# libAudioFlux/audioFlux

Hardware: NVIDIA H100
Metric: mfcc_frames_per_s (higher is better)
Workload: dtype f32

## Files before the change

### audioflux_b200/csrc/gen/gen_fft32.py

```python
#!/usr/bin/env python3
import math
import sys

import numpy as np


def bitrev5(k):
    return int("{:05b}".format(k)[::-1], 2)


def build_ops(n=32):
    ops = []
    span = n // 2
    while span >= 1:
        for base in range(0, n, 2 * span):
            for j in range(span):
                theta = 2 * math.pi * j / (2 * span)
                c, s = math.cos(theta), math.sin(theta)
                if j == 0:
                    kind = "one"
                elif 2 * j == span:
                    kind = "mi"
                elif 4 * j == span:
                    kind = "w8_1"
# ... 16 lines not shown
    bits = n.bit_length() - 1
    for i, j, kind, c, s in build_ops(n):
        u, v = x[i], x[j]
        x[i] = u + v
        x[j] = (u - v) * complex(c, -s)
    out = np.empty(n, dtype=np.complex128)
    for k in range(n):
        out[k] = x[bitrev(k, bits)]
    return out


def selfcheck():
    rng = np.random.default_rng(0)
    err = 0.0
    for n in (16, 32):
        x = rng.standard_normal(n) + 1j * rng.standard_normal(n)
        err = max(err, np.abs(run_numpy(x) - np.fft.fft(x)).max())
    x = rng.standard_normal(32) + 1j * rng.standard_normal(32)
    err = max(err, np.abs(run_numpy_fma(x) - np.fft.fft(x)).max())
    s = rng.standard_normal(64)
    err = max(err, np.abs(run_numpy_rfft64(s / 2) - np.fft.rfft(s)).max())
    w = rng.standard_normal(32) + 1j * rng.standard_normal(32)
    err = max(err, np.abs(run_numpy_fma_win(x, w) - np.fft.fft(x.real * w.real + 1j * x.imag * w.imag)).max())
    g, t = np.ones(32), np.zeros(32)
    for j in range(1, 32):
        g[j], t[j] = twiddle_gt(17 * j)
    err = max(err, np.abs(run_numpy_fma_tw(x, g, t) - np.fft.fft(x * g * (1 - 1j * t))).max())
    assert err < 1e-12, err
    return err


def lit(v):
    return repr(float(np.float32(v))) + "f"


def emit():
    out = []
    w = out.append
    w("// GENERATED by gen/gen_fft32.py -- do not edit.  32-point forward DFT on registers,")
    w("// complex values packed as c64 (see c64.cuh); X[k] is left at index AF_BR5(k) (5-bit reversal).")
    w("#pragma once")
    w('#include "c64.cuh"')
    w("#define AF_BR5(k) ((((k) & 1) << 4) | (((k) & 2) << 2) | ((k) & 4) | (((k) & 8) >> 2) | (((k) & 16) >> 4))")
    w("#define AF_BR4(k) ((((k) & 1) << 3) | (((k) & 2) << 1) | (((k) & 4) >> 1) | (((k) & 8) >> 3))")
    r2 = lit(math.sqrt(0.5))
    for n in (32, 16):
# ... 131 lines not shown
    for k in range(n // 4):
        mi1, g1, t1 = _twiddle(2 * math.pi * k / n)
        mi3, g3, t3 = _twiddle(2 * math.pi * 3 * k / n)
        a = o.rot(z1[k], t1)
        b = o.rot(z3[k], t3)
        if mi1:
            a = _mul_mi(a)
        if mi3:
            b = _mul_mi(b)
        if abs(g1) >= abs(g3):
            G, r = g1, _snap(g3 / g1)
            s, d = o.clin(b, r, a), o.clin(b, -r, a)
        else:
            G, r = g3, _snap(g1 / g3)
            s, d = o.clin(a, r, b), o.clin(a, r, (_neg(b[0]), _neg(b[1])))
        md = _mul_mi(d)
        out[k] = o.clin(s, G, u[k])
        out[k + n // 2] = o.clin(s, -G, u[k])
        out[k + n // 4] = o.clin(md, G, u[k + n // 4])
        out[k + 3 * n // 4] = o.clin(md, -G, u[k + n // 4])
    return out


def _inputs(n):
    return [((f"x{j}r", 1), (f"x{j}i", 1)) for j in range(n)]


def build_fma_fft32():
    o = _Ops()
    return o.ops, _split_radix(o, _inputs(32))


def build_fma_post64():
    o = _Ops()
    z = _inputs(32)
    out = [None] * 32
    for k in range(1, 16):
        zk, zc = z[k], (z[32 - k][0], _neg(z[32 - k][1]))
        ev = o.clin(zc, 1.0, zk)
        od = o.clin(zc, -1.0, zk)
        mi, g, t = _twiddle(2 * math.pi * k / 64 + math.pi / 2)
        a = o.rot(od, t)
        if mi:
            a = _mul_mi(a)
        out[k] = o.clin(a, g, ev)
        out[32 - k] = (o.lin(a[0], -g, ev[0]), o.lin(a[1], g, _neg(ev[1])))
    out[16] = (o.mul(z[16][0], 2.0), o.mul(z[16][1], -2.0))
    out[0] = (o.mul(o.lin(z[0][1], 1.0, z[0][0]), 2.0), o.mul(o.lin(z[0][1], -1.0, z[0][0]), 2.0))
    return o.ops, out


def build_fma_fft32_win():
    o = _Ops()
    xs = [((f"x{j}r", 1, f"w{j}r"), (f"x{j}i", 1, f"w{j}i")) for j in range(32)]
    return o.ops, _split_radix(o, xs)


def build_fma_fft32_tw():
    o = _Ops()
    xs = [((f"x0r", 1), (f"x0i", 1))]
    for j in range(1, 32):
        re = o.fmar((f"x{j}i", 1), f"t{j}", (f"x{j}r", 1))
        im = o.fmar((f"x{j}r", -1), f"t{j}", (f"x{j}i", 1))
        xs.append((re + (f"g{j}",), im + (f"g{j}",)))
    return o.ops, _split_radix(o, xs)


def twiddle_gt(m, n=2048):
    th = 2 * math.pi * m / n
    return math.cos(th), math.tan(th)


def fp32_op_count(ops):
    return len(ops)


def run_ops(ops, outs, x, dtype=np.float64, regs=None):
    f = np.float64 if dtype == np.float64 else np.float32
    env = {k: f(v) for k, v in (regs or {}).items()}
    for j, v in enumerate(x):
# ... 30 lines not shown
def run_numpy_fma_win(x, w, dtype=np.float64):
    ops, outs = build_fma_fft32_win()
    w = np.asarray(w, dtype=np.complex128)
    regs = {}
    for j in range(32):
        regs[f"w{j}r"], regs[f"w{j}i"] = w[j].real, w[j].imag
    return run_ops(ops, outs, np.asarray(x, dtype=np.complex128), dtype, regs)


def run_numpy_fma_tw(x, g, t, dtype=np.float64):
    ops, outs = build_fma_fft32_tw()
    regs = {}
    for j in range(1, 32):
        regs[f"g{j}"], regs[f"t{j}"] = g[j], t[j]
    return run_ops(ops, outs, np.asarray(x, dtype=np.complex128), dtype, regs)


def run_numpy_rfft64(s, dtype=np.float64):
    s = np.asarray(s, dtype=np.float64)
    x = s[0::2] + 1j * s[1::2]
    Z = run_numpy_fma(x, dtype)
    ops, outs = build_fma_post64()
    R = run_ops(ops, outs, Z, dtype)
    return np.concatenate([[R[0].real], R[1:32], [R[0].imag]])


def _operand(a):
    return ("-" if a[1] < 0 else "") + a[0]


def _emit_ops(w, ops):
    for op in ops:
        if op[0] == "add":
            a, b = op[2], op[3]
            if a[1] > 0 and b[1] < 0:
                w(f"    const float {op[1]} = __fsub_rn({a[0]}, {b[0]});")
            elif a[1] < 0 and b[1] > 0:
                w(f"    const float {op[1]} = __fsub_rn({b[0]}, {a[0]});")
            else:
                w(f"    const float {op[1]} = __fadd_rn({_operand(a)}, {_operand(b)});")
        elif op[0] == "mul":
            k = op[3] * op[2][1]
            w(f"    const float {op[1]} = __fmul_rn({op[2][0]}, {lit(k)});")
        elif op[0] == "mulr":
            w(f"    const float {op[1]} = __fmul_rn({_operand(op[2])}, {op[3]});")
        elif op[0] == "fmar":
# ... 3 lines not shown
            w(f"    const float {op[1]} = __fmaf_rn({op[2][0]}, {lit(k)}, {_operand(op[4])});")


def emit_fma():
    out = []
    w = out.append
    w("")
    w("// ---- FMA-oriented transforms (scalar FP32, one instruction per op; only the fused MFCC frame path uses them) ----")
    w("// Twiddles as u g (1 - i t), |t| <= 1, g folded into the consumer's FMAs; +-i and negation are operand modifiers.")
    w("// Results differ from af_fft32 in the last bits (different rounding sequence), deterministic.")
    ops, outs = build_fma_fft32()
    w("// Split-radix (decimation in time) 32-point forward DFT; X[k] is left at index AF_BR5(k), as af_fft32 leaves it.")
    w("__device__ __forceinline__ void af_fft32_fma(c64 (&z)[32]) {")
    for j in range(32):
        w(f"    float x{j}r, x{j}i; c_unpack(z[{j}], x{j}r, x{j}i);")
    _emit_ops(w, ops)
    for k, (r, i) in enumerate(outs):
        assert r[1] > 0 and i[1] > 0
        w(f"    z[{bitrev5(k)}] = c_pack({r[0]}, {i[0]});")
    w("}")
    w(f"// af_fft32_fma FP32 instruction count: {fp32_op_count(ops)}")
    ops, outs = build_fma_fft32_win()
    w("// af_fft32_fma of the windowed input (z[j].re w[32 j].re, z[j].im w[32 j].im): the window factors are applied inside")
    w("// the first butterflies (one FMUL + two FMAs per butterfly and component).")
    w("__device__ __forceinline__ void af_fft32_fma_win(c64 (&z)[32], const c64 *w) {")
    for j in range(32):
        w(f"    float x{j}r, x{j}i, w{j}r, w{j}i; c_unpack(z[{j}], x{j}r, x{j}i); c_unpack(w[{32 * j}], w{j}r, w{j}i);")
    _emit_ops(w, ops)
    for k, (r, i) in enumerate(outs):
        assert r[1] > 0 and i[1] > 0
        w(f"    z[{bitrev5(k)}] = c_pack({r[0]}, {i[0]});")
    w("}")
    w(f"// af_fft32_fma_win FP32 instruction count: {fp32_op_count(ops)}")
    ops, outs = build_fma_fft32_tw()
    w("// af_fft32_fma of z[j] g_j (1 - i t_j), (g_j, t_j) = tw[32 (j - 1)] for j = 1..31 (input 0 is taken as it is):")
    w("// two FMAs apply (1 - i t), g goes into the first butterflies as af_fft32_fma_win's window factors do.")
    w("__device__ __forceinline__ void af_fft32_fma_tw(c64 (&z)[32], const c64 *tw) {")
    w("    float x0r, x0i; c_unpack(z[0], x0r, x0i);")
    for j in range(1, 32):
        w(f"    float x{j}r, x{j}i, g{j}, t{j}; c_unpack(z[{j}], x{j}r, x{j}i); c_unpack(tw[{32 * (j - 1)}], g{j}, t{j});")
    _emit_ops(w, ops)
    for k, (r, i) in enumerate(outs):
        assert r[1] > 0 and i[1] > 0
        w(f"    z[{bitrev5(k)}] = c_pack({r[0]}, {i[0]});")
    w("}")
    w(f"// af_fft32_fma_tw FP32 instruction count: {fp32_op_count(ops)}")
    ops, outs = build_fma_post64()
    w("// Real 64-point DFT post-pass on the output of af_fft32_fma (Z[k] at AF_BR5(k)): R[k] at AF_BR5(k) for k = 1..31,")
    w("// (R[0], R[32]) packed at index 0; the window carries the factor 1/2.")
    w("__device__ __forceinline__ void af_rfft64_post_fma(c64 (&z)[32]) {")
    for j in range(32):
        w(f"    float x{j}r, x{j}i; c_unpack(z[{bitrev5(j)}], x{j}r, x{j}i);")
    _emit_ops(w, ops)
    for k, (r, i) in enumerate(outs):
        assert r[1] > 0 and i[1] > 0
        w(f"    z[{bitrev5(k)}] = c_pack({r[0]}, {i[0]});")
    w("}")
    w(f"// af_rfft64_post_fma FP32 instruction count: {fp32_op_count(ops)}")
    return out


if __name__ == "__main__":
    e = selfcheck()
    path = sys.argv[1] if len(sys.argv) > 1 else "../kernels/fft32_gen.cuh"
    with open(path, "w") as f:
        f.write(emit())
    n_r2 = sum(2 if kind in ("one", "mi") else 4 for _, _, kind, _, _ in build_ops(32))
    print(f"selfcheck err {e:.2e}; wrote {path}; FP32 instructions: af_fft32 {2 * n_r2}, "
          f"af_fft32_fma {fp32_op_count(build_fma_fft32()[0])}, af_fft32_fma_win {fp32_op_count(build_fma_fft32_win()[0])}, "
          f"af_fft32_fma_tw {fp32_op_count(build_fma_fft32_tw()[0])}, af_rfft64_post_fma {fp32_op_count(build_fma_post64()[0])}")
```

### audioflux_b200/csrc/kernels/fft32_gen.cuh

```cuda
#pragma once
#include "c64.cuh"
#define AF_BR5(k) ((((k) & 1) << 4) | (((k) & 2) << 2) | ((k) & 4) | (((k) & 8) >> 2) | (((k) & 16) >> 4))
#define AF_BR4(k) ((((k) & 1) << 3) | (((k) & 2) << 1) | (((k) & 4) >> 1) | (((k) & 8) >> 3))
__device__ __forceinline__ void af_fft32(c64 (&z)[32]) {
    c64 u, d;
    u = z[0]; d = c_sub(u, z[16]); z[0] = c_add(u, z[16]);
    z[16] = d;
    u = z[1]; d = c_sub(u, z[17]); z[1] = c_add(u, z[17]);
    z[17] = c_mul_cs(d, 0.9807852506637573f, 0.19509032368659973f);
    u = z[2]; d = c_sub(u, z[18]); z[2] = c_add(u, z[18]);
    z[18] = c_mul_cs(d, 0.9238795042037964f, 0.3826834261417389f);
    u = z[3]; d = c_sub(u, z[19]); z[3] = c_add(u, z[19]);
    z[19] = c_mul_cs(d, 0.8314695954322815f, 0.5555702447891235f);
    u = z[4]; d = c_sub(u, z[20]); z[4] = c_add(u, z[20]);
    z[20] = c_scale(c_add(d, c_mul_mi(d)), 0.7071067690849304f);
    u = z[5]; d = c_sub(u, z[21]); z[5] = c_add(u, z[21]);
    z[21] = c_mul_cs(d, 0.5555702447891235f, 0.8314695954322815f);
    u = z[6]; d = c_sub(u, z[22]); z[6] = c_add(u, z[22]);
    z[22] = c_mul_cs(d, 0.3826834261417389f, 0.9238795042037964f);
    u = z[7]; d = c_sub(u, z[23]); z[7] = c_add(u, z[23]);
    z[23] = c_mul_cs(d, 0.19509032368659973f, 0.9807852506637573f);
    u = z[8]; d = c_sub(u, z[24]); z[8] = c_add(u, z[24]);
    z[24] = c_mul_mi(d);
    u = z[9]; d = c_sub(u, z[25]); z[9] = c_add(u, z[25]);
// ... 1887 lines not shown
    z[10] = c_pack(v97, v98);
    z[26] = c_pack(v107, v108);
    z[6] = c_pack(v117, v118);
    z[22] = c_pack(v127, v128);
    z[14] = c_pack(v137, v138);
    z[30] = c_pack(v147, v148);
    z[1] = c_pack(v151, v152);
    z[17] = c_pack(v149, v150);
    z[9] = c_pack(v139, v140);
    z[25] = c_pack(v129, v130);
    z[5] = c_pack(v119, v120);
    z[21] = c_pack(v109, v110);
    z[13] = c_pack(v99, v100);
    z[29] = c_pack(v89, v90);
    z[3] = c_pack(v79, v80);
    z[19] = c_pack(v69, v70);
    z[11] = c_pack(v59, v60);
    z[27] = c_pack(v49, v50);
    z[7] = c_pack(v39, v40);
    z[23] = c_pack(v29, v30);
    z[15] = c_pack(v19, v20);
    z[31] = c_pack(v9, v10);
}
```

### audioflux_b200/csrc/kernels/mfcc_fused2.cu

```cuda
#include <string.h>
#include "mfcc_common.cuh"
#include "fft32_gen.cuh"

namespace {

constexpr int kN = 2048;
constexpr int kBins = 1025;
constexpr int kPairs = 513;
constexpr int kFW = 13;
constexpr int kBW = 4;
constexpr int kDW = 2;
constexpr int kEW = kBW;
constexpr int kThreads = (kFW + 1 + kBW + kDW) * 32;
constexpr int kProducerWarp = 13;
__device__ __forceinline__ int bank_warp_index(int warp) { return warp >= 14 && warp <= 18 && warp != 16 ? warp - 14 - (warp > 16) : -1; }
__device__ __forceinline__ int dct_warp_index(int warp) { return warp == 16 || warp == 19 ? (warp - 16) / 3 : -1; }
constexpr int kMaxNum = 128;
constexpr int kLPitch = 132;
constexpr int kMaxTab = 1408;
constexpr int kMaxPieces = 256;
constexpr int kMaxPass = kMaxPieces / (kEW * 32);
constexpr int kSpecPitch = 17;
constexpr int kPitchPairs = kFW | 1;
constexpr int kTileFloats = kPairs * kPitchPairs * 2;
// ... 366 lines not shown
        float *col = sP + sb * kTileFloats + 2 * warp;

        af_mbar_wait(&fullBar[stage], stagePhase);

        c64 z[32];
        if (active) {
            const float *sp = span + (size_t)stage * p.spanFloats + warp * p.hop + lane;
#pragma unroll
            for (int m = 0; m < 32; m++) z[m] = c_pack(sp[64 * m], sp[64 * m + 32]);
        }
        __syncwarp();
        if (lane == 0) af_mbar_arrive(&emptyBar[stage]);
        if (++stage == p.stages) { stage = 0; stagePhase ^= 1u; }
        if (!active) {
            af_mbar_wait(&pEmpty[sb], ((uint32_t)(it >> 1) & 1u) ^ 1u);
            if (lane == 0) {
                af_mbar_arrive(&specFull[sb]);
                af_mbar_arrive(&cDone[sb]);
                af_mbar_arrive(&pFull[sb]);
            }
            continue;
        }

        af_fft32_fma_win(z, sWinC + lane);
        af_rfft64_post_fma(z);
        af_mbar_wait(&pEmpty[sb], ((uint32_t)(it >> 1) & 1u) ^ 1u);
        sSpec[((size_t)sb * 32 + lane) * kSpecPitch + warp] = z[0];
        __syncwarp();
        if (lane == 0) af_mbar_arrive(&specFull[sb]);

        {
            float yr[32], yi[32];
            float *tw = col + trWrite;
            const float2 *row = reinterpret_cast<const float2 *>(col) + trRead;
#pragma unroll
            for (int k1 = 1; k1 < 32; k1++) c_unpack(z[AF_BR5(k1)], yr[k1], yi[k1]);
#pragma unroll
            for (int k1 = 1; k1 < 32; k1++) tw[(k1 - 1) * 2 * pitch] = yr[k1];
            __syncwarp();
#pragma unroll
            for (int j = 0; j < 16; j++) { const float2 v = row[j * kTrRows * pitch]; yr[2 * j] = v.x; yr[2 * j + 1] = v.y; }
            __syncwarp();
#pragma unroll
            for (int k1 = 1; k1 < 32; k1++) tw[(k1 - 1) * 2 * pitch] = yi[k1];
            __syncwarp();
#pragma unroll
            for (int j = 0; j < 16; j++) {
                const float2 v = row[j * kTrRows * pitch];
                z[2 * j] = c_pack(yr[2 * j], v.x);
                z[2 * j + 1] = c_pack(yr[2 * j + 1], v.y);
            }
            __syncwarp();
            if (lane == 0) af_mbar_arrive(&cDone[sb]);
        }
        af_fft32_fma_tw(z, sTwC + lane);
        if (lane) {
            if (p.dataType == SpectralData_Mag) {
#pragma unroll
                for (int k2 = 0; k2 < 32; k2++) {
// ... 179 lines not shown
    Intervals *iv = static_cast<Intervals *>(malloc(sizeof(Intervals)));
    float4 *tab = static_cast<float4 *>(malloc(sizeof(float4) * kMaxTab));
    unsigned desc[kMaxNum + 4];
    PiecePlan *pc = static_cast<PiecePlan *>(malloc(sizeof(PiecePlan)));
    const int ok = iv && tab && pc && build_intervals2(bank, num, iv) && build_table(bank, num, iv, desc, tab) >= 0 &&
                   plan_pieces(num, desc, pc) > 0;
    free(iv); free(tab); free(pc);
    return ok;
}

void af_mfcc2_plan_free(void *plan) { free_plan(static_cast<Plan *>(plan)); }

int af_mfcc2_plan_build(void **planOut, int fftLength, int num, int ccNum, const float *window, const float *bank,
                        const float *dct , int dataType) {
    *planOut = NULL;
    if (!af_mfcc2_supported(fftLength, num, ccNum, bank)) return af_fail(AF_ERR_UNSUPPORTED, "fused MFCC v2 plan: unsupported configuration");
    Plan *pl = static_cast<Plan *>(calloc(1, sizeof(Plan)));
    if (!pl) return AF_ERR_NOMEM;
    pl->num = num; pl->ccNum = ccNum; pl->dataType = dataType;
    pl->ct = af_mfcc_ct(ccNum);
    int rc = AF_OK;

    float2 *wp = static_cast<float2 *>(malloc(sizeof(float2) * 1024));
    for (int m = 0; m < 32; m++)
        for (int l = 0; l < 32; l++) wp[m * 32 + l] = make_float2(0.5f * window[64 * m + l], 0.5f * window[64 * m + 32 + l]);
    rc = af_dev_upload(reinterpret_cast<void **>(&pl->dWinPairs), wp, sizeof(float2) * 1024);
    for (int n2 = 1; n2 <= kTwRows; n2++)
        for (int k1 = 0; k1 < 32; k1++) {
            const double a = 2.0 * M_PI * (double)(n2 * k1) / 2048.0;
            wp[(n2 - 1) * 32 + k1] = make_float2((float)cos(a), (float)tan(a));
        }
    if (rc == AF_OK) rc = af_dev_upload(reinterpret_cast<void **>(&pl->dTw), wp, sizeof(float2) * kTwRows * 32);
    free(wp);

    Intervals *iv = static_cast<Intervals *>(malloc(sizeof(Intervals)));
    pl->tab = static_cast<float4 *>(malloc(sizeof(float4) * kMaxTab));
    if (!iv || !pl->tab) { free(iv); free_plan(pl); return AF_ERR_NOMEM; }
    build_intervals2(bank, num, iv);
    pl->tabLen = build_table(bank, num, iv, pl->ivDesc, pl->tab);
    free(iv);
    for (int i = num + 2; i < kMaxNum + 4; i++) pl->ivDesc[i] = pl->ivDesc[num + 1];
    {
        PiecePlan *pc = static_cast<PiecePlan *>(malloc(sizeof(PiecePlan)));
        if (!pc || plan_pieces(num, pl->ivDesc, pc) <= 0) { free(pc); free_plan(pl); return af_fail(AF_ERR_UNSUPPORTED, "fused MFCC v2 plan: no piece plan"); }
        pl->nPass = pc->nPass; pl->nPieces = pc->nPieces; pl->lmax = pc->lmax; pl->firstPass2 = pc->firstPass2;
        memcpy(pl->pieceDesc, pc->pieceDesc, sizeof(pl->pieceDesc));
        memcpy(pl->piecePrefix, pc->prefix, sizeof(pl->piecePrefix));
        memcpy(pl->assign, pc->assign, sizeof(pl->assign));
// ... 83 lines not shown
```

Before: 240.2 million.

## Replace packed complex FFT32 plus real post-pass with direct split-radix real FFT64

Stage B of the fused MFCC kernel used to run a 32-point complex FFT on packed sample pairs followed by a separate real-64 post-pass. It now runs one generated split-radix real 64-point DFT with the window applied inside the first butterflies, and writes outputs in natural order so the transpose no longer needs bit-reversed indexing. The aim is fewer FP32 instructions and lower register pressure in the per-warp FFT. The window-pair table layout on the host changes to match, and rounding differs slightly from the old path.

```diff
diff --git a/audioflux_b200/csrc/gen/gen_fft32.py b/audioflux_b200/csrc/gen/gen_fft32.py
--- a/audioflux_b200/csrc/gen/gen_fft32.py
+++ b/audioflux_b200/csrc/gen/gen_fft32.py
@@ -62,6 +62,8 @@
     err = max(err, np.abs(run_numpy_rfft64(s / 2) - np.fft.rfft(s)).max())
     w = rng.standard_normal(32) + 1j * rng.standard_normal(32)
     err = max(err, np.abs(run_numpy_fma_win(x, w) - np.fft.fft(x.real * w.real + 1j * x.imag * w.imag)).max())
+    w = rng.standard_normal(64)
+    err = max(err, np.abs(run_numpy_rfft64_win(s, w) - np.fft.rfft(s * w)).max())
     g, t = np.ones(32), np.zeros(32)
     for j in range(1, 32):
         g[j], t[j] = twiddle_gt(17 * j)
@@ -239,6 +241,48 @@
     return out
 
 
+def _real_split_radix(o, xs):
+    n = len(xs)
+    if n == 1:
+        return [xs[0]]
+    if n == 2:
+        return [o.lin(xs[1], 1.0, xs[0]), o.lin(xs[1], -1.0, xs[0])]
+    u = _real_split_radix(o, xs[0::2])
+    z1 = _real_split_radix(o, xs[1::4])
+    z3 = _real_split_radix(o, xs[3::4])
+    out = [None] * (n // 2 + 1)
+    a, nb = o.lin(z1[0], 1.0, z3[0]), o.lin(z1[0], -1.0, z3[0])
+    out[0], out[n // 2] = o.lin(a, 1.0, u[0]), o.lin(a, -1.0, u[0])
+    out[n // 4] = (u[n // 4], nb)
+    if n >= 8:
+        e, r = n // 8, math.sqrt(0.5)
+        p, q = o.lin(z3[e], -1.0, z1[e]), o.lin(z3[e], 1.0, z1[e])
+        ue = u[e]
+        out[e] = (o.lin(p, r, ue[0]), o.lin(q, -r, ue[1]))
+        out[3 * e] = (o.lin(p, -r, ue[0]), o.lin(q, -r, _neg(ue[1])))
+    for k in range(1, n // 8):
+        mi1, g1, t1 = _twiddle(2 * math.pi * k / n)
+        mi3, g3, t3 = _twiddle(2 * math.pi * 3 * k / n)
+        a = o.rot(z1[k], t1)
+        b = o.rot(z3[k], t3)
+        if mi1:
+            a = _mul_mi(a)
+        if mi3:
+            b = _mul_mi(b)
+        if abs(g1) >= abs(g3):
+            G, r = g1, _snap(g3 / g1)
+            s, d = o.clin(b, r, a), o.clin(b, -r, a)
+        else:
+            G, r = g3, _snap(g1 / g3)
+            s, d = o.clin(a, r, b), o.clin(a, r, (_neg(b[0]), _neg(b[1])))
+        uk, uq = u[k], u[n // 4 - k]
+        out[k] = o.clin(s, G, uk)
+        out[n // 2 - k] = (o.lin(s[0], -G, uk[0]), o.lin(s[1], G, _neg(uk[1])))
+        out[n // 4 + k] = (o.lin(d[1], G, uq[0]), o.lin(d[0], -G, _neg(uq[1])))
+        out[n // 4 - k] = (o.lin(d[1], -G, uq[0]), o.lin(d[0], -G, uq[1]))
+    return out
+
+
 def _inputs(n):
     return [((f"x{j}r", 1), (f"x{j}i", 1)) for j in range(n)]
 
@@ -273,6 +317,13 @@
     return o.ops, _split_radix(o, xs)
 
 
+def build_fma_rfft64_win():
+    o = _Ops()
+    xs = [(f"x{n // 2}{'ri'[n & 1]}", 1, f"w{n}") for n in range(64)]
+    R = _real_split_radix(o, xs)
+    return o.ops, [(R[0], R[32])] + R[1:32]
+
+
 def build_fma_fft32_tw():
     o = _Ops()
     xs = [((f"x0r", 1), (f"x0i", 1))]
@@ -349,6 +400,14 @@
     Z = run_numpy_fma(x, dtype)
     ops, outs = build_fma_post64()
     R = run_ops(ops, outs, Z, dtype)
+    return np.concatenate([[R[0].real], R[1:32], [R[0].imag]])
+
+
+def run_numpy_rfft64_win(s, w, dtype=np.float64):
+    ops, outs = build_fma_rfft64_win()
+    s, w = np.asarray(s, dtype=np.float64), np.asarray(w, dtype=np.float64)
+    regs = {f"w{n}": w[n] for n in range(64)}
+    R = run_ops(ops, outs, s[0::2] + 1j * s[1::2], dtype, regs)
     return np.concatenate([[R[0].real], R[1:32], [R[0].imag]])
 
 
@@ -398,7 +457,8 @@
     w(f"// af_fft32_fma FP32 instruction count: {fp32_op_count(ops)}")
     ops, outs = build_fma_fft32_win()
     w("// af_fft32_fma of the windowed input (z[j].re w[32 j].re, z[j].im w[32 j].im): the window factors are applied inside")
-    w("// the first butterflies (one FMUL + two FMAs per butterfly and component).")
+    w("// the first butterflies (one FMUL + two FMAs per butterfly and component).  With af_rfft64_post_fma it makes the real")
+    w("// 64-point DFT of packed sample pairs; no kernel calls the pair now (the fused MFCC stage B is af_rfft64_fma_win).")
     w("__device__ __forceinline__ void af_fft32_fma_win(c64 (&z)[32], const c64 *w) {")
     for j in range(32):
         w(f"    float x{j}r, x{j}i, w{j}r, w{j}i; c_unpack(z[{j}], x{j}r, x{j}i); c_unpack(w[{32 * j}], w{j}r, w{j}i);")
@@ -423,7 +483,8 @@
     w(f"// af_fft32_fma_tw FP32 instruction count: {fp32_op_count(ops)}")
     ops, outs = build_fma_post64()
     w("// Real 64-point DFT post-pass on the output of af_fft32_fma (Z[k] at AF_BR5(k)): R[k] at AF_BR5(k) for k = 1..31,")
-    w("// (R[0], R[32]) packed at index 0; the window carries the factor 1/2.")
+    w("// (R[0], R[32]) packed at index 0; the window carries the factor 1/2.  Not called by any kernel now (see")
+    w("// af_fft32_fma_win).")
     w("__device__ __forceinline__ void af_rfft64_post_fma(c64 (&z)[32]) {")
     for j in range(32):
         w(f"    float x{j}r, x{j}i; c_unpack(z[{bitrev5(j)}], x{j}r, x{j}i);")
@@ -433,6 +494,19 @@
         w(f"    z[{bitrev5(k)}] = c_pack({r[0]}, {i[0]});")
     w("}")
     w(f"// af_rfft64_post_fma FP32 instruction count: {fp32_op_count(ops)}")
+    ops, outs = build_fma_rfft64_win()
+    w("// Split-radix (decimation in time) real 64-point DFT of the windowed samples s[n] w[n], packed as z[j] = (s[2j],")
+    w("// s[2j+1]), with the window pairs w[32 n] = (w[n], w[n + 32]) of the first butterflies (s[n] with s[n + 32]); the")
+    w("// window factors are applied inside them.  Leaves R[k] at z[k] for k = 1..31 and the real pair (R[0], R[32]) at z[0].")
+    w("__device__ __forceinline__ void af_rfft64_fma_win(c64 (&z)[32], const c64 *w) {")
+    for j in range(32):
+        w(f"    float x{j}r, x{j}i, w{j}, w{j + 32}; c_unpack(z[{j}], x{j}r, x{j}i); c_unpack(w[{32 * j}], w{j}, w{j + 32});")
+    _emit_ops(w, ops)
+    for k, (r, i) in enumerate(outs):
+        assert r[1] > 0 and i[1] > 0
+        w(f"    z[{k}] = c_pack({r[0]}, {i[0]});")
+    w("}")
+    w(f"// af_rfft64_fma_win FP32 instruction count: {fp32_op_count(ops)}")
     return out
 
 
@@ -444,4 +518,5 @@
     n_r2 = sum(2 if kind in ("one", "mi") else 4 for _, _, kind, _, _ in build_ops(32))
     print(f"selfcheck err {e:.2e}; wrote {path}; FP32 instructions: af_fft32 {2 * n_r2}, "
           f"af_fft32_fma {fp32_op_count(build_fma_fft32()[0])}, af_fft32_fma_win {fp32_op_count(build_fma_fft32_win()[0])}, "
-          f"af_fft32_fma_tw {fp32_op_count(build_fma_fft32_tw()[0])}, af_rfft64_post_fma {fp32_op_count(build_fma_post64()[0])}")
+          f"af_fft32_fma_tw {fp32_op_count(build_fma_fft32_tw()[0])}, af_rfft64_post_fma {fp32_op_count(build_fma_post64()[0])}, "
+          f"af_rfft64_fma_win {fp32_op_count(build_fma_rfft64_win()[0])}")
diff --git a/audioflux_b200/csrc/kernels/fft32_gen.cuh b/audioflux_b200/csrc/kernels/fft32_gen.cuh
--- a/audioflux_b200/csrc/kernels/fft32_gen.cuh
+++ b/audioflux_b200/csrc/kernels/fft32_gen.cuh
@@ -1933,3 +1933,495 @@
     z[15] = c_pack(v19, v20);
     z[31] = c_pack(v9, v10);
 }
+__device__ __forceinline__ void af_rfft64_fma_win(c64 (&z)[32], const c64 *w) {
+    float x0r, x0i, w0, w32; c_unpack(z[0], x0r, x0i); c_unpack(w[0], w0, w32);
+    float x1r, x1i, w1, w33; c_unpack(z[1], x1r, x1i); c_unpack(w[32], w1, w33);
+    float x2r, x2i, w2, w34; c_unpack(z[2], x2r, x2i); c_unpack(w[64], w2, w34);
+    float x3r, x3i, w3, w35; c_unpack(z[3], x3r, x3i); c_unpack(w[96], w3, w35);
+    float x4r, x4i, w4, w36; c_unpack(z[4], x4r, x4i); c_unpack(w[128], w4, w36);
+    float x5r, x5i, w5, w37; c_unpack(z[5], x5r, x5i); c_unpack(w[160], w5, w37);
+    float x6r, x6i, w6, w38; c_unpack(z[6], x6r, x6i); c_unpack(w[192], w6, w38);
+    float x7r, x7i, w7, w39; c_unpack(z[7], x7r, x7i); c_unpack(w[224], w7, w39);
+    float x8r, x8i, w8, w40; c_unpack(z[8], x8r, x8i); c_unpack(w[256], w8, w40);
+    float x9r, x9i, w9, w41; c_unpack(z[9], x9r, x9i); c_unpack(w[288], w9, w41);
+    float x10r, x10i, w10, w42; c_unpack(z[10], x10r, x10i); c_unpack(w[320], w10, w42);
+    float x11r, x11i, w11, w43; c_unpack(z[11], x11r, x11i); c_unpack(w[352], w11, w43);
+    float x12r, x12i, w12, w44; c_unpack(z[12], x12r, x12i); c_unpack(w[384], w12, w44);
+    float x13r, x13i, w13, w45; c_unpack(z[13], x13r, x13i); c_unpack(w[416], w13, w45);
+    float x14r, x14i, w14, w46; c_unpack(z[14], x14r, x14i); c_unpack(w[448], w14, w46);
+    float x15r, x15i, w15, w47; c_unpack(z[15], x15r, x15i); c_unpack(w[480], w15, w47);
+    float x16r, x16i, w16, w48; c_unpack(z[16], x16r, x16i); c_unpack(w[512], w16, w48);
+    float x17r, x17i, w17, w49; c_unpack(z[17], x17r, x17i); c_unpack(w[544], w17, w49);
+    float x18r, x18i, w18, w50; c_unpack(z[18], x18r, x18i); c_unpack(w[576], w18, w50);
+    float x19r, x19i, w19, w51; c_unpack(z[19], x19r, x19i); c_unpack(w[608], w19, w51);
+    float x20r, x20i, w20, w52; c_unpack(z[20], x20r, x20i); c_unpack(w[640], w20, w52);
+    float x21r, x21i, w21, w53; c_unpack(z[21], x21r, x21i); c_unpack(w[672], w21, w53);
+    float x22r, x22i, w22, w54; c_unpack(z[22], x22r, x22i); c_unpack(w[704], w22, w54);
+    float x23r, x23i, w23, w55; c_unpack(z[23], x23r, x23i); c_unpack(w[736], w23, w55);
+    float x24r, x24i, w24, w56; c_unpack(z[24], x24r, x24i); c_unpack(w[768], w24, w56);
+    float x25r, x25i, w25, w57; c_unpack(z[25], x25r, x25i); c_unpack(w[800], w25, w57);
+    float x26r, x26i, w26, w58; c_unpack(z[26], x26r, x26i); c_unpack(w[832], w26, w58);
+    float x27r, x27i, w27, w59; c_unpack(z[27], x27r, x27i); c_unpack(w[864], w27, w59);
+    float x28r, x28i, w28, w60; c_unpack(z[28], x28r, x28i); c_unpack(w[896], w28, w60);
+    float x29r, x29i, w29, w61; c_unpack(z[29], x29r, x29i); c_unpack(w[928], w29, w61);
+    float x30r, x30i, w30, w62; c_unpack(z[30], x30r, x30i); c_unpack(w[960], w30, w62);
+    float x31r, x31i, w31, w63; c_unpack(z[31], x31r, x31i); c_unpack(w[992], w31, w63);
+    const float v1 = __fmul_rn(x0r, w0);
+    const float v2 = __fmaf_rn(x16r, w32, v1);
+    const float v3 = __fmaf_rn(-x16r, w32, v1);
+    const float v4 = __fmul_rn(x24r, w48);
+    const float v5 = __fmaf_rn(x8r, w16, v4);
+    const float v6 = __fmaf_rn(-x8r, w16, v4);
+    const float v7 = __fadd_rn(v5, v2);
+    const float v8 = __fsub_rn(v2, v5);
+    const float v9 = __fmul_rn(x4r, w8);
+    const float v10 = __fmaf_rn(x20r, w40, v9);
+    const float v11 = __fmaf_rn(-x20r, w40, v9);
+    const float v12 = __fmul_rn(x12r, w24);
+    const float v13 = __fmaf_rn(x28r, w56, v12);
+    const float v14 = __fmaf_rn(-x28r, w56, v12);
+    const float v15 = __fadd_rn(v10, v13);
+    const float v16 = __fsub_rn(v13, v10);
+    const float v17 = __fadd_rn(v15, v7);
+    const float v18 = __fsub_rn(v7, v15);
+    const float v19 = __fsub_rn(v11, v14);
+    const float v20 = __fadd_rn(v14, v11);
+    const float v21 = __fmaf_rn(v19, 0.7071067690849304f, v3);
+    const float v22 = __fmaf_rn(v20, -0.7071067690849304f, v6);
+    const float v23 = __fmaf_rn(v19, -0.7071067690849304f, v3);
+    const float v24 = __fmaf_rn(v20, -0.7071067690849304f, -v6);
+    const float v25 = __fmul_rn(x2r, w4);
+    const float v26 = __fmaf_rn(x18r, w36, v25);
+    const float v27 = __fmaf_rn(-x18r, w36, v25);
+    const float v28 = __fmul_rn(x26r, w52);
+    const float v29 = __fmaf_rn(x10r, w20, v28);
+    const float v30 = __fmaf_rn(-x10r, w20, v28);
+    const float v31 = __fadd_rn(v29, v26);
+    const float v32 = __fsub_rn(v26, v29);
+    const float v33 = __fmul_rn(x6r, w12);
+    const float v34 = __fmaf_rn(x22r, w44, v33);
+    const float v35 = __fmaf_rn(-x22r, w44, v33);
+    const float v36 = __fmul_rn(x30r, w60);
+    const float v37 = __fmaf_rn(x14r, w28, v36);
+    const float v38 = __fmaf_rn(-x14r, w28, v36);
+    const float v39 = __fadd_rn(v37, v34);
+    const float v40 = __fsub_rn(v34, v37);
+    const float v41 = __fadd_rn(v31, v39);
+    const float v42 = __fsub_rn(v39, v31);
+    const float v43 = __fadd_rn(v41, v17);
+    const float v44 = __fsub_rn(v17, v41);
+    const float v45 = __fsub_rn(v32, v40);
+    const float v46 = __fadd_rn(v40, v32);
+    const float v47 = __fmaf_rn(v45, 0.7071067690849304f, v8);
+    const float v48 = __fmaf_rn(v46, -0.7071067690849304f, v16);
+    const float v49 = __fmaf_rn(v45, -0.7071067690849304f, v8);
+    const float v50 = __fmaf_rn(v46, -0.7071067690849304f, -v16);
+    const float v51 = __fmaf_rn(v30, 0.4142135679721832f, v27);
+    const float v52 = __fmaf_rn(v27, -0.4142135679721832f, v30);
+    const float v53 = __fmaf_rn(v38, -0.4142135679721832f, v35);
+    const float v54 = __fmaf_rn(v35, 0.4142135679721832f, v38);
+    const float v55 = __fadd_rn(v54, v51);
+    const float v56 = __fsub_rn(v52, v53);
+    const float v57 = __fsub_rn(v51, v54);
+    const float v58 = __fadd_rn(v53, v52);
+    const float v59 = __fmaf_rn(v55, 0.9238795042037964f, v21);
+    const float v60 = __fmaf_rn(v56, 0.9238795042037964f, v22);
+    const float v61 = __fmaf_rn(v55, -0.9238795042037964f, v21);
+    const float v62 = __fmaf_rn(v56, 0.9238795042037964f, -v22);
+    const float v63 = __fmaf_rn(v58, 0.9238795042037964f, v23);
+    const float v64 = __fmaf_rn(v57, -0.9238795042037964f, -v24);
+    const float v65 = __fmaf_rn(v58, -0.9238795042037964f, v23);
+    const float v66 = __fmaf_rn(v57, -0.9238795042037964f, v24);
+    const float v67 = __fmul_rn(x1r, w2);
+    const float v68 = __fmaf_rn(x17r, w34, v67);
+    const float v69 = __fmaf_rn(-x17r, w34, v67);
+    const float v70 = __fmul_rn(x25r, w50);
+    const float v71 = __fmaf_rn(x9r, w18, v70);
+    const float v72 = __fmaf_rn(-x9r, w18, v70);
+    const float v73 = __fadd_rn(v71, v68);
+    const float v74 = __fsub_rn(v68, v71);
+    const float v75 = __fmul_rn(x5r, w10);
+    const float v76 = __fmaf_rn(x21r, w42, v75);
+    const float v77 = __fmaf_rn(-x21r, w42, v75);
+    const float v78 = __fmul_rn(x13r, w26);
+    const float v79 = __fmaf_rn(x29r, w58, v78);
+    const float v80 = __fmaf_rn(-x29r, w58, v78);
+    const float v81 = __fadd_rn(v76, v79);
+    const float v82 = __fsub_rn(v79, v76);
+    const float v83 = __fadd_rn(v81, v73);
+    const float v84 = __fsub_rn(v73, v81);
+    const float v85 = __fsub_rn(v77, v80);
+    const float v86 = __fadd_rn(v80, v77);
+    const float v87 = __fmaf_rn(v85, 0.7071067690849304f, v69);
+    const float v88 = __fmaf_rn(v86, -0.7071067690849304f, v72);
+    const float v89 = __fmaf_rn(v85, -0.7071067690849304f, v69);
+    const float v90 = __fmaf_rn(v86, -0.7071067690849304f, -v72);
+    const float v91 = __fmul_rn(x3r, w6);
+    const float v92 = __fmaf_rn(x19r, w38, v91);
+    const float v93 = __fmaf_rn(-x19r, w38, v91);
+    const float v94 = __fmul_rn(x27r, w54);
+    const float v95 = __fmaf_rn(x11r, w22, v94);
+    const float v96 = __fmaf_rn(-x11r, w22, v94);
+    const float v97 = __fadd_rn(v95, v92);
+    const float v98 = __fsub_rn(v92, v95);
+    const float v99 = __fmul_rn(x7r, w14);
+    const float v100 = __fmaf_rn(x23r, w46, v99);
+    const float v101 = __fmaf_rn(-x23r, w46, v99);
+    const float v102 = __fmul_rn(x15r, w30);
+    const float v103 = __fmaf_rn(x31r, w62, v102);
+    const float v104 = __fmaf_rn(-x31r, w62, v102);
+    const float v105 = __fadd_rn(v100, v103);
+    const float v106 = __fsub_rn(v103, v100);
+    const float v107 = __fadd_rn(v105, v97);
+    const float v108 = __fsub_rn(v97, v105);
+    const float v109 = __fsub_rn(v101, v104);
+    const float v110 = __fadd_rn(v104, v101);
+    const float v111 = __fmaf_rn(v109, 0.7071067690849304f, v93);
+    const float v112 = __fmaf_rn(v110, -0.7071067690849304f, v96);
+    const float v113 = __fmaf_rn(v109, -0.7071067690849304f, v93);
+    const float v114 = __fmaf_rn(v110, -0.7071067690849304f, -v96);
+    const float v115 = __fadd_rn(v83, v107);
+    const float v116 = __fsub_rn(v107, v83);
+    const float v117 = __fadd_rn(v115, v43);
+    const float v118 = __fsub_rn(v43, v115);
+    const float v119 = __fsub_rn(v84, v108);
+    const float v120 = __fadd_rn(v108, v84);
+    const float v121 = __fmaf_rn(v119, 0.7071067690849304f, v18);
+    const float v122 = __fmaf_rn(v120, -0.7071067690849304f, v42);
+    const float v123 = __fmaf_rn(v119, -0.7071067690849304f, v18);
+    const float v124 = __fmaf_rn(v120, -0.7071067690849304f, -v42);
+    const float v125 = __fmaf_rn(v88, 0.1989123672246933f, v87);
+    const float v126 = __fmaf_rn(v87, -0.1989123672246933f, v88);
+    const float v127 = __fmaf_rn(v112, 0.6681786179542542f, v111);
+    const float v128 = __fmaf_rn(v111, -0.6681786179542542f, v112);
+    const float v129 = __fmaf_rn(v127, 0.8477590680122375f, v125);
+    const float v130 = __fmaf_rn(v128, 0.8477590680122375f, v126);
+    const float v131 = __fmaf_rn(v127, -0.8477590680122375f, v125);
+    const float v132 = __fmaf_rn(v128, -0.8477590680122375f, v126);
+    const float v133 = __fmaf_rn(v129, 0.9807852506637573f, v59);
+    const float v134 = __fmaf_rn(v130, 0.9807852506637573f, v60);
+    const float v135 = __fmaf_rn(v129, -0.9807852506637573f, v59);
+    const float v136 = __fmaf_rn(v130, 0.9807852506637573f, -v60);
+    const float v137 = __fmaf_rn(v132, 0.9807852506637573f, v61);
+    const float v138 = __fmaf_rn(v131, -0.9807852506637573f, -v62);
+    const float v139 = __fmaf_rn(v132, -0.9807852506637573f, v61);
+    const float v140 = __fmaf_rn(v131, -0.9807852506637573f, v62);
+    const float v141 = __fmaf_rn(v82, 0.4142135679721832f, v74);
+    const float v142 = __fmaf_rn(v74, -0.4142135679721832f, v82);
+    const float v143 = __fmaf_rn(v106, -0.4142135679721832f, v98);
+    const float v144 = __fmaf_rn(v98, 0.4142135679721832f, v106);
+    const float v145 = __fadd_rn(v144, v141);
+    const float v146 = __fsub_rn(v142, v143);
+    const float v147 = __fsub_rn(v141, v144);
+    const float v148 = __fadd_rn(v143, v142);
+    const float v149 = __fmaf_rn(v145, 0.9238795042037964f, v47);
+    const float v150 = __fmaf_rn(v146, 0.9238795042037964f, v48);
+    const float v151 = __fmaf_rn(v145, -0.9238795042037964f, v47);
+    const float v152 = __fmaf_rn(v146, 0.9238795042037964f, -v48);
+    const float v153 = __fmaf_rn(v148, 0.9238795042037964f, v49);
+    const float v154 = __fmaf_rn(v147, -0.9238795042037964f, -v50);
+    const float v155 = __fmaf_rn(v148, -0.9238795042037964f, v49);
+    const float v156 = __fmaf_rn(v147, -0.9238795042037964f, v50);
+    const float v157 = __fmaf_rn(v90, 0.6681786179542542f, v89);
+    const float v158 = __fmaf_rn(v89, -0.6681786179542542f, v90);
+    const float v159 = __fmaf_rn(v114, 0.1989123672246933f, v113);
+    const float v160 = __fmaf_rn(v113, -0.1989123672246933f, v114);
+    const float v161 = __fmaf_rn(v157, 0.8477590680122375f, v160);
+    const float v162 = __fmaf_rn(v158, 0.8477590680122375f, -v159);
+    const float v163 = __fmaf_rn(v157, 0.8477590680122375f, -v160);
+    const float v164 = __fmaf_rn(v158, 0.8477590680122375f, v159);
+    const float v165 = __fmaf_rn(v161, 0.9807852506637573f, v65);
+    const float v166 = __fmaf_rn(v162, 0.9807852506637573f, v66);
+    const float v167 = __fmaf_rn(v161, -0.9807852506637573f, v65);
+    const float v168 = __fmaf_rn(v162, 0.9807852506637573f, -v66);
+    const float v169 = __fmaf_rn(v164, 0.9807852506637573f, v63);
+    const float v170 = __fmaf_rn(v163, -0.9807852506637573f, -v64);
+    const float v171 = __fmaf_rn(v164, -0.9807852506637573f, v63);
+    const float v172 = __fmaf_rn(v163, -0.9807852506637573f, v64);
+    const float v173 = __fmul_rn(x0i, w1);
+    const float v174 = __fmaf_rn(x16i, w33, v173);
+    const float v175 = __fmaf_rn(-x16i, w33, v173);
+    const float v176 = __fmul_rn(x24i, w49);
+    const float v177 = __fmaf_rn(x8i, w17, v176);
+    const float v178 = __fmaf_rn(-x8i, w17, v176);
+    const float v179 = __fadd_rn(v177, v174);
+    const float v180 = __fsub_rn(v174, v177);
+    const float v181 = __fmul_rn(x4i, w9);
+    const float v182 = __fmaf_rn(x20i, w41, v181);
+    const float v183 = __fmaf_rn(-x20i, w41, v181);
+    const float v184 = __fmul_rn(x12i, w25);
+    const float v185 = __fmaf_rn(x28i, w57, v184);
+    const float v186 = __fmaf_rn(-x28i, w57, v184);
+    const float v187 = __fadd_rn(v182, v185);
+    const float v188 = __fsub_rn(v185, v182);
+    const float v189 = __fadd_rn(v187, v179);
+    const float v190 = __fsub_rn(v179, v187);
+    const float v191 = __fsub_rn(v183, v186);
+    const float v192 = __fadd_rn(v186, v183);
+    const float v193 = __fmaf_rn(v191, 0.7071067690849304f, v175);
+    const float v194 = __fmaf_rn(v192, -0.7071067690849304f, v178);
+    const float v195 = __fmaf_rn(v191, -0.7071067690849304f, v175);
+    const float v196 = __fmaf_rn(v192, -0.7071067690849304f, -v178);
+    const float v197 = __fmul_rn(x2i, w5);
+    const float v198 = __fmaf_rn(x18i, w37, v197);
+    const float v199 = __fmaf_rn(-x18i, w37, v197);
+    const float v200 = __fmul_rn(x26i, w53);
+    const float v201 = __fmaf_rn(x10i, w21, v200);
+    const float v202 = __fmaf_rn(-x10i, w21, v200);
+    const float v203 = __fadd_rn(v201, v198);
+    const float v204 = __fsub_rn(v198, v201);
+    const float v205 = __fmul_rn(x6i, w13);
+    const float v206 = __fmaf_rn(x22i, w45, v205);
+    const float v207 = __fmaf_rn(-x22i, w45, v205);
+    const float v208 = __fmul_rn(x30i, w61);
+    const float v209 = __fmaf_rn(x14i, w29, v208);
+    const float v210 = __fmaf_rn(-x14i, w29, v208);
+    const float v211 = __fadd_rn(v209, v206);
+    const float v212 = __fsub_rn(v206, v209);
+    const float v213 = __fadd_rn(v203, v211);
+    const float v214 = __fsub_rn(v211, v203);
+    const float v215 = __fadd_rn(v213, v189);
+    const float v216 = __fsub_rn(v189, v213);
+    const float v217 = __fsub_rn(v204, v212);
+    const float v218 = __fadd_rn(v212, v204);
+    const float v219 = __fmaf_rn(v217, 0.7071067690849304f, v180);
+    const float v220 = __fmaf_rn(v218, -0.7071067690849304f, v188);
+    const float v221 = __fmaf_rn(v217, -0.7071067690849304f, v180);
+    const float v222 = __fmaf_rn(v218, -0.7071067690849304f, -v188);
+    const float v223 = __fmaf_rn(v202, 0.4142135679721832f, v199);
+    const float v224 = __fmaf_rn(v199, -0.4142135679721832f, v202);
+    const float v225 = __fmaf_rn(v210, -0.4142135679721832f, v207);
+    const float v226 = __fmaf_rn(v207, 0.4142135679721832f, v210);
+    const float v227 = __fadd_rn(v226, v223);
+    const float v228 = __fsub_rn(v224, v225);
+    const float v229 = __fsub_rn(v223, v226);
+    const float v230 = __fadd_rn(v225, v224);
+    const float v231 = __fmaf_rn(v227, 0.9238795042037964f, v193);
+    const float v232 = __fmaf_rn(v228, 0.9238795042037964f, v194);
+    const float v233 = __fmaf_rn(v227, -0.9238795042037964f, v193);
+    const float v234 = __fmaf_rn(v228, 0.9238795042037964f, -v194);
+    const float v235 = __fmaf_rn(v230, 0.9238795042037964f, v195);
+    const float v236 = __fmaf_rn(v229, -0.9238795042037964f, -v196);
+    const float v237 = __fmaf_rn(v230, -0.9238795042037964f, v195);
+    const float v238 = __fmaf_rn(v229, -0.9238795042037964f, v196);
+    const float v239 = __fmul_rn(x1i, w3);
+    const float v240 = __fmaf_rn(x17i, w35, v239);
+    const float v241 = __fmaf_rn(-x17i, w35, v239);
+    const float v242 = __fmul_rn(x25i, w51);
+    const float v243 = __fmaf_rn(x9i, w19, v242);
+    const float v244 = __fmaf_rn(-x9i, w19, v242);
+    const float v245 = __fadd_rn(v243, v240);
+    const float v246 = __fsub_rn(v240, v243);
+    const float v247 = __fmul_rn(x5i, w11);
+    const float v248 = __fmaf_rn(x21i, w43, v247);
+    const float v249 = __fmaf_rn(-x21i, w43, v247);
+    const float v250 = __fmul_rn(x13i, w27);
+    const float v251 = __fmaf_rn(x29i, w59, v250);
+    const float v252 = __fmaf_rn(-x29i, w59, v250);
+    const float v253 = __fadd_rn(v248, v251);
+    const float v254 = __fsub_rn(v251, v248);
+    const float v255 = __fadd_rn(v253, v245);
+    const float v256 = __fsub_rn(v245, v253);
+    const float v257 = __fsub_rn(v249, v252);
+    const float v258 = __fadd_rn(v252, v249);
+    const float v259 = __fmaf_rn(v257, 0.7071067690849304f, v241);
+    const float v260 = __fmaf_rn(v258, -0.7071067690849304f, v244);
+    const float v261 = __fmaf_rn(v257, -0.7071067690849304f, v241);
+    const float v262 = __fmaf_rn(v258, -0.7071067690849304f, -v244);
+    const float v263 = __fmul_rn(x3i, w7);
+    const float v264 = __fmaf_rn(x19i, w39, v263);
+    const float v265 = __fmaf_rn(-x19i, w39, v263);
+    const float v266 = __fmul_rn(x27i, w55);
+    const float v267 = __fmaf_rn(x11i, w23, v266);
+    const float v268 = __fmaf_rn(-x11i, w23, v266);
+    const float v269 = __fadd_rn(v267, v264);
+    const float v270 = __fsub_rn(v264, v267);
+    const float v271 = __fmul_rn(x7i, w15);
+    const float v272 = __fmaf_rn(x23i, w47, v271);
+    const float v273 = __fmaf_rn(-x23i, w47, v271);
+    const float v274 = __fmul_rn(x31i, w63);
+    const float v275 = __fmaf_rn(x15i, w31, v274);
+    const float v276 = __fmaf_rn(-x15i, w31, v274);
+    const float v277 = __fadd_rn(v275, v272);
+    const float v278 = __fsub_rn(v272, v275);
+    const float v279 = __fadd_rn(v269, v277);
+    const float v280 = __fsub_rn(v277, v269);
+    const float v281 = __fadd_rn(v279, v255);
+    const float v282 = __fsub_rn(v255, v279);
+    const float v283 = __fsub_rn(v270, v278);
+    const float v284 = __fadd_rn(v278, v270);
+    const float v285 = __fmaf_rn(v283, 0.7071067690849304f, v246);
+    const float v286 = __fmaf_rn(v284, -0.7071067690849304f, v254);
+    const float v287 = __fmaf_rn(v283, -0.7071067690849304f, v246);
+    const float v288 = __fmaf_rn(v284, -0.7071067690849304f, -v254);
+    const float v289 = __fmaf_rn(v268, 0.4142135679721832f, v265);
+    const float v290 = __fmaf_rn(v265, -0.4142135679721832f, v268);
+    const float v291 = __fmaf_rn(v276, -0.4142135679721832f, v273);
+    const float v292 = __fmaf_rn(v273, 0.4142135679721832f, v276);
+    const float v293 = __fadd_rn(v292, v289);
+    const float v294 = __fsub_rn(v290, v291);
+    const float v295 = __fsub_rn(v289, v292);
+    const float v296 = __fadd_rn(v291, v290);
+    const float v297 = __fmaf_rn(v293, 0.9238795042037964f, v259);
+    const float v298 = __fmaf_rn(v294, 0.9238795042037964f, v260);
+    const float v299 = __fmaf_rn(v293, -0.9238795042037964f, v259);
+    const float v300 = __fmaf_rn(v294, 0.9238795042037964f, -v260);
+    const float v301 = __fmaf_rn(v296, 0.9238795042037964f, v261);
+    const float v302 = __fmaf_rn(v295, -0.9238795042037964f, -v262);
+    const float v303 = __fmaf_rn(v296, -0.9238795042037964f, v261);
+    const float v304 = __fmaf_rn(v295, -0.9238795042037964f, v262);
+    const float v305 = __fadd_rn(v215, v281);
+    const float v306 = __fsub_rn(v281, v215);
+    const float v307 = __fadd_rn(v305, v117);
+    const float v308 = __fsub_rn(v117, v305);
+    const float v309 = __fsub_rn(v216, v282);
+    const float v310 = __fadd_rn(v282, v216);
+    const float v311 = __fmaf_rn(v309, 0.7071067690849304f, v44);
+    const float v312 = __fmaf_rn(v310, -0.7071067690849304f, v116);
+    const float v313 = __fmaf_rn(v309, -0.7071067690849304f, v44);
+    const float v314 = __fmaf_rn(v310, -0.7071067690849304f, -v116);
+    const float v315 = __fmaf_rn(v232, 0.09849140048027039f, v231);
+    const float v316 = __fmaf_rn(v231, -0.09849140048027039f, v232);
+    const float v317 = __fmaf_rn(v298, 0.3033466935157776f, v297);
+    const float v318 = __fmaf_rn(v297, -0.3033466935157776f, v298);
+    const float v319 = __fmaf_rn(v317, 0.9615705609321594f, v315);
+    const float v320 = __fmaf_rn(v318, 0.9615705609321594f, v316);
+    const float v321 = __fmaf_rn(v317, -0.9615705609321594f, v315);
+    const float v322 = __fmaf_rn(v318, -0.9615705609321594f, v316);
+    const float v323 = __fmaf_rn(v319, 0.9951847195625305f, v133);
+    const float v324 = __fmaf_rn(v320, 0.9951847195625305f, v134);
+    const float v325 = __fmaf_rn(v319, -0.9951847195625305f, v133);
+    const float v326 = __fmaf_rn(v320, 0.9951847195625305f, -v134);
+    const float v327 = __fmaf_rn(v322, 0.9951847195625305f, v135);
+    const float v328 = __fmaf_rn(v321, -0.9951847195625305f, -v136);
+    const float v329 = __fmaf_rn(v322, -0.9951847195625305f, v135);
+    const float v330 = __fmaf_rn(v321, -0.9951847195625305f, v136);
+    const float v331 = __fmaf_rn(v220, 0.1989123672246933f, v219);
+    const float v332 = __fmaf_rn(v219, -0.1989123672246933f, v220);
+    const float v333 = __fmaf_rn(v286, 0.6681786179542542f, v285);
+    const float v334 = __fmaf_rn(v285, -0.6681786179542542f, v286);
+    const float v335 = __fmaf_rn(v333, 0.8477590680122375f, v331);
+    const float v336 = __fmaf_rn(v334, 0.8477590680122375f, v332);
+    const float v337 = __fmaf_rn(v333, -0.8477590680122375f, v331);
+    const float v338 = __fmaf_rn(v334, -0.8477590680122375f, v332);
+    const float v339 = __fmaf_rn(v335, 0.9807852506637573f, v149);
+    const float v340 = __fmaf_rn(v336, 0.9807852506637573f, v150);
+    const float v341 = __fmaf_rn(v335, -0.9807852506637573f, v149);
+    const float v342 = __fmaf_rn(v336, 0.9807852506637573f, -v150);
+    const float v343 = __fmaf_rn(v338, 0.9807852506637573f, v151);
+    const float v344 = __fmaf_rn(v337, -0.9807852506637573f, -v152);
+    const float v345 = __fmaf_rn(v338, -0.9807852506637573f, v151);
+    const float v346 = __fmaf_rn(v337, -0.9807852506637573f, v152);
+    const float v347 = __fmaf_rn(v238, 0.3033466935157776f, v237);
+    const float v348 = __fmaf_rn(v237, -0.3033466935157776f, v238);
+    const float v349 = __fmaf_rn(v304, -0.8206787705421448f, v303);
+    const float v350 = __fmaf_rn(v303, 0.8206787705421448f, v304);
+    const float v351 = __fmaf_rn(v350, 0.8077937960624695f, v347);
+    const float v352 = __fmaf_rn(v349, -0.8077937960624695f, v348);
+    const float v353 = __fmaf_rn(v350, -0.8077937960624695f, v347);
+    const float v354 = __fmaf_rn(v349, 0.8077937960624695f, v348);
+    const float v355 = __fmaf_rn(v351, 0.9569403529167175f, v165);
+    const float v356 = __fmaf_rn(v352, 0.9569403529167175f, v166);
+    const float v357 = __fmaf_rn(v351, -0.9569403529167175f, v165);
+    const float v358 = __fmaf_rn(v352, 0.9569403529167175f, -v166);
+    const float v359 = __fmaf_rn(v354, 0.9569403529167175f, v167);
+    const float v360 = __fmaf_rn(v353, -0.9569403529167175f, -v168);
+    const float v361 = __fmaf_rn(v354, -0.9569403529167175f, v167);
+    const float v362 = __fmaf_rn(v353, -0.9569403529167175f, v168);
+    const float v363 = __fmaf_rn(v214, 0.4142135679721832f, v190);
+    const float v364 = __fmaf_rn(v190, -0.4142135679721832f, v214);
+    const float v365 = __fmaf_rn(v280, -0.4142135679721832f, v256);
+    const float v366 = __fmaf_rn(v256, 0.4142135679721832f, v280);
+    const float v367 = __fadd_rn(v366, v363);
+    const float v368 = __fsub_rn(v364, v365);
+    const float v369 = __fsub_rn(v363, v366);
+    const float v370 = __fadd_rn(v365, v364);
+    const float v371 = __fmaf_rn(v367, 0.9238795042037964f, v121);
+    const float v372 = __fmaf_rn(v368, 0.9238795042037964f, v122);
+    const float v373 = __fmaf_rn(v367, -0.9238795042037964f, v121);
+    const float v374 = __fmaf_rn(v368, 0.9238795042037964f, -v122);
+    const float v375 = __fmaf_rn(v370, 0.9238795042037964f, v123);
+    const float v376 = __fmaf_rn(v369, -0.9238795042037964f, -v124);
+    const float v377 = __fmaf_rn(v370, -0.9238795042037964f, v123);
+    const float v378 = __fmaf_rn(v369, -0.9238795042037964f, v124);
+    const float v379 = __fmaf_rn(v236, 0.534511148929596f, v235);
+    const float v380 = __fmaf_rn(v235, -0.534511148929596f, v236);
+    const float v381 = __fmaf_rn(v302, -0.09849140048027039f, v301);
+    const float v382 = __fmaf_rn(v301, 0.09849140048027039f, v302);
+    const float v383 = __fmaf_rn(v379, 0.8861885070800781f, v382);
+    const float v384 = __fmaf_rn(v380, 0.8861885070800781f, -v381);
+    const float v385 = __fmaf_rn(v379, 0.8861885070800781f, -v382);
+    const float v386 = __fmaf_rn(v380, 0.8861885070800781f, v381);
+    const float v387 = __fmaf_rn(v383, 0.9951847195625305f, v171);
+    const float v388 = __fmaf_rn(v384, 0.9951847195625305f, v172);
+    const float v389 = __fmaf_rn(v383, -0.9951847195625305f, v171);
+    const float v390 = __fmaf_rn(v384, 0.9951847195625305f, -v172);
+    const float v391 = __fmaf_rn(v386, 0.9951847195625305f, v169);
+    const float v392 = __fmaf_rn(v385, -0.9951847195625305f, -v170);
+    const float v393 = __fmaf_rn(v386, -0.9951847195625305f, v169);
+    const float v394 = __fmaf_rn(v385, -0.9951847195625305f, v170);
+    const float v395 = __fmaf_rn(v222, 0.6681786179542542f, v221);
+    const float v396 = __fmaf_rn(v221, -0.6681786179542542f, v222);
+    const float v397 = __fmaf_rn(v288, 0.1989123672246933f, v287);
+    const float v398 = __fmaf_rn(v287, -0.1989123672246933f, v288);
+    const float v399 = __fmaf_rn(v395, 0.8477590680122375f, v398);
+    const float v400 = __fmaf_rn(v396, 0.8477590680122375f, -v397);
+    const float v401 = __fmaf_rn(v395, 0.8477590680122375f, -v398);
+    const float v402 = __fmaf_rn(v396, 0.8477590680122375f, v397);
+    const float v403 = __fmaf_rn(v399, 0.9807852506637573f, v155);
+    const float v404 = __fmaf_rn(v400, 0.9807852506637573f, v156);
+    const float v405 = __fmaf_rn(v399, -0.9807852506637573f, v155);
+    const float v406 = __fmaf_rn(v400, 0.9807852506637573f, -v156);
+    const float v407 = __fmaf_rn(v402, 0.9807852506637573f, v153);
+    const float v408 = __fmaf_rn(v401, -0.9807852506637573f, -v154);
+    const float v409 = __fmaf_rn(v402, -0.9807852506637573f, v153);
+    const float v410 = __fmaf_rn(v401, -0.9807852506637573f, v154);
+    const float v411 = __fmaf_rn(v234, 0.8206787705421448f, v233);
+    const float v412 = __fmaf_rn(v233, -0.8206787705421448f, v234);
+    const float v413 = __fmaf_rn(v300, 0.534511148929596f, v299);
+    const float v414 = __fmaf_rn(v299, -0.534511148929596f, v300);
+    const float v415 = __fmaf_rn(v411, 0.8765073418617249f, v414);
+    const float v416 = __fmaf_rn(v412, 0.8765073418617249f, -v413);
+    const float v417 = __fmaf_rn(v411, 0.8765073418617249f, -v414);
+    const float v418 = __fmaf_rn(v412, 0.8765073418617249f, v413);
+    const float v419 = __fmaf_rn(v415, 0.8819212913513184f, v139);
+    const float v420 = __fmaf_rn(v416, 0.8819212913513184f, v140);
+    const float v421 = __fmaf_rn(v415, -0.8819212913513184f, v139);
+    const float v422 = __fmaf_rn(v416, 0.8819212913513184f, -v140);
+    const float v423 = __fmaf_rn(v418, 0.8819212913513184f, v137);
+    const float v424 = __fmaf_rn(v417, -0.8819212913513184f, -v138);
+    const float v425 = __fmaf_rn(v418, -0.8819212913513184f, v137);
+    const float v426 = __fmaf_rn(v417, -0.8819212913513184f, v138);
+    z[0] = c_pack(v307, v308);
+    z[1] = c_pack(v323, v324);
+    z[2] = c_pack(v339, v340);
+    z[3] = c_pack(v355, v356);
+    z[4] = c_pack(v371, v372);
+    z[5] = c_pack(v387, v388);
+    z[6] = c_pack(v403, v404);
+    z[7] = c_pack(v419, v420);
+    z[8] = c_pack(v311, v312);
+    z[9] = c_pack(v425, v426);
+    z[10] = c_pack(v409, v410);
+    z[11] = c_pack(v393, v394);
+    z[12] = c_pack(v377, v378);
+    z[13] = c_pack(v361, v362);
+    z[14] = c_pack(v345, v346);
+    z[15] = c_pack(v329, v330);
+    z[16] = c_pack(v118, v306);
+    z[17] = c_pack(v327, v328);
+    z[18] = c_pack(v343, v344);
+    z[19] = c_pack(v359, v360);
+    z[20] = c_pack(v375, v376);
+    z[21] = c_pack(v391, v392);
+    z[22] = c_pack(v407, v408);
+    z[23] = c_pack(v423, v424);
+    z[24] = c_pack(v313, v314);
+    z[25] = c_pack(v421, v422);
+    z[26] = c_pack(v405, v406);
+    z[27] = c_pack(v389, v390);
+    z[28] = c_pack(v373, v374);
+    z[29] = c_pack(v357, v358);
+    z[30] = c_pack(v341, v342);
+    z[31] = c_pack(v325, v326);
+}
diff --git a/audioflux_b200/csrc/kernels/mfcc_fused2.cu b/audioflux_b200/csrc/kernels/mfcc_fused2.cu
--- a/audioflux_b200/csrc/kernels/mfcc_fused2.cu
+++ b/audioflux_b200/csrc/kernels/mfcc_fused2.cu
@@ -412,8 +412,7 @@
             continue;
         }
 
-        af_fft32_fma_win(z, sWinC + lane);
-        af_rfft64_post_fma(z);
+        af_rfft64_fma_win(z, sWinC + lane);
         af_mbar_wait(&pEmpty[sb], ((uint32_t)(it >> 1) & 1u) ^ 1u);
         sSpec[((size_t)sb * 32 + lane) * kSpecPitch + warp] = z[0];
         __syncwarp();
@@ -424,7 +423,7 @@
             float *tw = col + trWrite;
             const float2 *row = reinterpret_cast<const float2 *>(col) + trRead;
 #pragma unroll
-            for (int k1 = 1; k1 < 32; k1++) c_unpack(z[AF_BR5(k1)], yr[k1], yi[k1]);
+            for (int k1 = 1; k1 < 32; k1++) c_unpack(z[k1], yr[k1], yi[k1]);
 #pragma unroll
             for (int k1 = 1; k1 < 32; k1++) tw[(k1 - 1) * 2 * pitch] = yr[k1];
             __syncwarp();
@@ -650,8 +649,8 @@
     int rc = AF_OK;
 
     float2 *wp = static_cast<float2 *>(malloc(sizeof(float2) * 1024));
-    for (int m = 0; m < 32; m++)
-        for (int l = 0; l < 32; l++) wp[m * 32 + l] = make_float2(0.5f * window[64 * m + l], 0.5f * window[64 * m + 32 + l]);
+    for (int n = 0; n < 32; n++)
+        for (int l = 0; l < 32; l++) wp[n * 32 + l] = make_float2(window[32 * n + l], window[32 * n + 1024 + l]);
     rc = af_dev_upload(reinterpret_cast<void **>(&pl->dWinPairs), wp, sizeof(float2) * 1024);
     for (int n2 = 1; n2 <= kTwRows; n2++)
         for (int k1 = 0; k1 < 32; k1++) {
```

After: 245.4 million, median of 6. +2.2%, better.
